# jinkyu032/TPDM

Hardware: NVIDIA B200
Metric: images/sec/box, SD3-M 1024^2 TPDM sampling (higher is better)
Workload: dtype bf16

## Files before the change

### include/tpdm_b200.h

```cpp
#ifndef TPDM_B200_H_
#define TPDM_B200_H_

#include <stddef.h>
#include <stdint.h>

#ifdef __cplusplus
extern "C" {
#endif

#define TPDM_ABI_VERSION 3

typedef enum tpdm_status {
  TPDM_OK = 0,
  TPDM_ERR_ARG = -1,
  TPDM_ERR_SHAPE = -2,
  TPDM_ERR_CUDA = -3,
  TPDM_ERR_STATE = -4,
  TPDM_ERR_NOMEM = -5
} tpdm_status;

typedef struct tpdm_config {
  int32_t num_layers;
  int32_t num_heads;
  int32_t head_dim;
// ... 198 lines not shown
int tpdm_vae_set_weights(tpdm_vae* vae, const tpdm_vae_weights* w);
size_t tpdm_vae_workspace_bytes(const tpdm_vae* vae, int latent_h, int latent_w);
int tpdm_vae_decode(tpdm_vae* vae, const float* latents, int apply_scaling, int batch, int latent_h, int latent_w,
                    void* workspace, size_t workspace_bytes, float* image, unsigned char* rgb, void* stream);

long long tpdm_launch_count(int reset);
int tpdm_profile_start(int max_records);
int tpdm_profile_stop(double* ms, double* flops, long long* count, int n_classes);
long long tpdm_profile_dropped(void);

int tpdm_gemm_bf16(const void* A, const void* W, const float* bias, const float* gate, void* out, int batch, int rows,
                   int N, int K, int epi, void* stream);
int tpdm_joint_attention(const void* qkv, void* out, int Bt, int S, int H, int dp, int head_dim, int q_rows, void* stream);
int tpdm_attention_redo_count(void);
long long tpdm_attention_redo_total(void);
int tpdm_conv3x3_nhwc(const void* x, const void* w, const float* bias, float* out, int batch, int g, int C, int N,
                      void* stream);
int tpdm_conv3x3_wgrad(const void* dyt, const void* x_shifted_nchw, float* dw, int samples, int g, int C, int M, void* stream);
int tpdm_ln_modulate(const float* x, const float* shift, const float* scale, int mod_stride, void* out_bf16, int batch,
                     int rows, int D, void* stream);

#ifdef __cplusplus
}
#endif
#endif
```

### tpdm_b200/_lib.py

```python
from __future__ import annotations

import ctypes as C
import os

HERE = os.path.dirname(os.path.abspath(__file__))
LIB_PATH = os.environ.get("TPDM_B200_LIB", os.path.join(HERE, "libtpdm_b200.so"))

c_float_p = C.POINTER(C.c_float)
vp = C.c_void_p

TPDM_OK, TPDM_ERR_ARG, TPDM_ERR_SHAPE, TPDM_ERR_CUDA, TPDM_ERR_STATE, TPDM_ERR_NOMEM = 0, -1, -2, -3, -4, -5


class TpdmConfig(C.Structure):
    _fields_ = [(n, C.c_int32) for n in (
        "num_layers", "num_heads", "head_dim", "joint_attention_dim", "pooled_projection_dim", "in_channels",
        "out_channels", "patch_size", "pos_embed_max_size", "qk_norm", "tpm_channels", "prediction_type", "relative")
    ] + [("min_sigma", C.c_float), ("epsilon", C.c_float), ("tpm_epsilon", C.c_float), ("dual_attention_mask", C.c_uint64)]


BLOCK_FIELDS = ("qkv_w", "qkv_b", "cqkv_w", "cqkv_b", "out_w", "out_b", "cout_w", "cout_b", "ff1_w", "ff1_b", "ff2_w",
                "ff2_b", "cff1_w", "cff1_b", "cff2_w", "cff2_b", "norm_q", "norm_k", "norm_added_q", "norm_added_k",
                "qkv2_w", "qkv2_b", "out2_w", "out2_b", "norm_q2", "norm_k2")

# ... 75 lines not shown
    "tpdm_rollout_shaping": (C.c_int, [vp, vp, vp, vp, vp, C.c_int, C.c_int, C.c_int, C.c_int, C.c_float, C.c_float, C.c_int, C.c_int,
                                       vp, vp, vp, vp, vp]),
    "tpdm_ppo_clip_loss": (C.c_int, [vp, vp, vp, vp, C.c_int, C.c_int, C.c_float, C.c_float, C.c_int, C.c_int, C.c_float, C.c_float, vp, vp, vp,
                                     vp, vp]),
    "tpdm_beta_logprob": (C.c_int, [vp, vp, C.c_int, C.c_int, C.c_float, C.c_float, C.c_int, C.c_int, C.c_float, vp, vp, vp]),
    "tpdm_adamw_step": (C.c_int, [vp, vp, vp, vp, C.c_longlong, C.c_float, C.c_float, C.c_float, C.c_float, C.c_float, C.c_float, C.c_int,
                                  C.c_float, vp, vp, C.c_longlong, vp, vp]),
    "tpdm_launch_count": (C.c_longlong, [C.c_int]),
    "tpdm_profile_start": (C.c_int, [C.c_int]),
    "tpdm_profile_dropped": (C.c_longlong, []),
    "tpdm_profile_stop": (C.c_int, [C.POINTER(C.c_double), C.POINTER(C.c_double), C.POINTER(C.c_longlong), C.c_int]),
    "tpdm_gemm_bf16": (C.c_int, [vp, vp, vp, vp, vp, C.c_int, C.c_int, C.c_int, C.c_int, C.c_int, vp]),
    "tpdm_joint_attention": (C.c_int, [vp, vp, C.c_int, C.c_int, C.c_int, C.c_int, C.c_int, C.c_int, vp]),
    "tpdm_attention_redo_count": (C.c_int, []),
    "tpdm_attention_redo_total": (C.c_longlong, []),
    "tpdm_conv3x3_nhwc": (C.c_int, [vp, vp, vp, vp, C.c_int, C.c_int, C.c_int, C.c_int, vp]),
    "tpdm_conv3x3_wgrad": (C.c_int, [vp, vp, vp, C.c_int, C.c_int, C.c_int, C.c_int, vp]),
    "tpdm_ln_modulate": (C.c_int, [vp, vp, vp, C.c_int, vp, C.c_int, C.c_int, C.c_int, vp]),
}

_lib = None


def load() -> C.CDLL:
    global _lib
    if _lib is None:
        if not os.path.exists(LIB_PATH):
            raise RuntimeError(f"{LIB_PATH} is missing: build it with `python -m tpdm_b200.build` "
                               "(tpdm_b200 has no CPU / PyTorch fallback)")
        lib = C.CDLL(LIB_PATH)
# ... 34 lines not shown
```

### tpdm_b200/csrc/api.cu

```cuda
#include <string.h>

#include <new>
#include <cstdlib>
#include <vector>

#include "host.h"
#include "kernels.h"

using namespace tpdm;

struct tpdm_ctx {
  tpdm_config cfg;
  tpdm_weights w;
  std::vector<tpdm_block_weights> blocks;
  bool has_weights = false, has_mmdit = false, has_tpm = false;
  int D = 0, dp = 0, Dp = 0, R = 0, device = 0;
  std::vector<int> mod_off;
  bool any_dual = false;
  bool dual(int i) const { return i < 64 && ((cfg.dual_attention_mask >> i) & 1ull) != 0; }
  int norm1_rows(int i) const { return (dual(i) ? 9 : 6) * D; }
};

namespace {

// ... 748 lines not shown
  TPDM_TRY(gemm_op_init(&op, A, K, static_cast<long long>(rows) * K, rows, batch, K, W, N, epi, out, static_cast<long long>(rows) * N, N, bias,
                        gate, N));
  return gemm_launch(&op, 1, static_cast<cudaStream_t>(stream));
}

int tpdm_joint_attention(const void* qkv, void* out, int Bt, int S, int H, int dp, int head_dim, int q_rows, void* stream) {
  TPDM_CHECK(qkv && out, TPDM_ERR_ARG, "tpdm_joint_attention: null argument");
  AttnOp op;
  TPDM_TRY(attn_op_init(&op, qkv, Bt, S, H, dp, head_dim, out));
  if (q_rows > 0 && q_rows < S) op.q_tiles = (q_rows + 127) / 128;
  return attn_launch(&op, static_cast<cudaStream_t>(stream));
}

int tpdm_attention_redo_count(void) { return attn_redo_count(); }
long long tpdm_attention_redo_total(void) { return attn_redo_total(); }

int tpdm_conv3x3_nhwc(const void* x, const void* w, const float* bias, float* out, int batch, int g, int C, int N, void* stream) {
  TPDM_CHECK(x && w && out, TPDM_ERR_ARG, "tpdm_conv3x3_nhwc: null argument");
  GemmOp op;
  TPDM_TRY(gemm_op_init_conv3x3(&op, x, batch, g, C, w, N, EPI_BIAS_F32, out, N, bias));
  return gemm_launch(&op, 1, static_cast<cudaStream_t>(stream));
}

int tpdm_conv3x3_wgrad(const void* dyt, const void* x_shifted_nchw, float* dw, int samples, int g, int C, int M, void* stream) {
  TPDM_CHECK(dyt && x_shifted_nchw && dw, TPDM_ERR_ARG, "tpdm_conv3x3_wgrad: null argument");
  GemmOp op;
  TPDM_TRY(gemm_op_init_conv3x3_wgrad(&op, dyt, x_shifted_nchw, samples, g, C, M, dw));
  return gemm_launch(&op, 1, static_cast<cudaStream_t>(stream));
}

// ... 9 lines not shown
```

### tpdm_b200/csrc/attention_tcgen05.cu

```cuda
#include <cuda_bf16.h>

#include <stdlib.h>

#include <type_traits>

#include "common.cuh"
#include "host.h"

namespace tpdm {

namespace {

constexpr int kFastThreads = 384;
constexpr int kQT = 128;
constexpr int kKT = 128;
constexpr int kChunk = 32;
constexpr int kKVStages = 2;
constexpr float kRescaleThreshold = 32.0f;
constexpr int kPolyEvery = 4;
#ifdef TPDM_ATTN_TRACE
__device__ long long g_attn_trace[3][2048];
#define ATRACE(role, idx)                                                                       \
  do {                                                                                          \
    if (trace_on && lane == 0 && (idx) < 2048) g_attn_trace[role][idx] = clock64();             \
  } while (0)
#define STRACE(e)                                                                               \
  do {                                                                                          \
    if (warp == 4) ATRACE(0, 8 * j + (e));                                                      \
  } while (0)
__device__ long long g_cta_trace[2][16];
#define CTRACE(idx)                                                                             \
  do {                                                                                          \
    if (ctr >= 0 && threadIdx.x == 128) g_cta_trace[ctr][idx] = clock64();                      \
  } while (0)
#else
#define ATRACE(role, idx)
#define STRACE(e)
#define CTRACE(idx)
#endif

__device__ unsigned long long g_redo_total;

template <int DP>
struct AttnSmem {
  static constexpr int kTile = kQT * DP * 2;
  static constexpr int kQOff = 0;
  static constexpr int kKOff = kTile;
  static constexpr int kVOff = kKOff + kKVStages * kTile;
  static constexpr int kBarOff = kVOff + kKVStages * kTile;
  static constexpr int kTotal = kBarOff + 256 + 1024;
  static constexpr uint32_t kTmemCols = DP == 64 ? 256 : 512;
  static constexpr uint32_t kSCol = 0;
  static constexpr uint32_t kPCol = 128;
  static constexpr uint32_t kOCol = 192;
};

template <int DP>
struct AttnBars {
  uint64_t *q_full, *k_full, *v_full, *k_empty, *v_empty, *s_full, *s_free, *p_full, *pv_done;
  uint32_t* tmem_slot;
  __device__ explicit AttnBars(uint8_t* smem) {
    uint64_t* bars = reinterpret_cast<uint64_t*>(smem + AttnSmem<DP>::kBarOff);
    q_full = bars + 0;
    k_full = bars + 1;
    v_full = k_full + kKVStages;
    k_empty = v_full + kKVStages;
    v_empty = k_empty + kKVStages;
    s_full = v_empty + kKVStages;
    s_free = s_full + 1;
    p_full = s_free + 1;
    pv_done = p_full + 2;
    tmem_slot = reinterpret_cast<uint32_t*>(pv_done + 1);
  }
  static constexpr int kCount = 1 + 4 * kKVStages + 5;
  __device__ void init(bool again, uint32_t s_free_count) const {
    if (again) {
      for (int i = 0; i < kCount; ++i) mbar_inval(q_full + i);
    }
    mbar_init(q_full, 1);
    for (int i = 0; i < kKVStages; ++i) {
      mbar_init(&k_full[i], 1);
      mbar_init(&v_full[i], 1);
      mbar_init(&k_empty[i], 1);
      mbar_init(&v_empty[i], 1);
    }
    mbar_init(s_full, 1);
    mbar_init(s_free, s_free_count);
    mbar_init(&p_full[0], 4);
    mbar_init(&p_full[1], 4);
    mbar_init(pv_done, 1);
    fence_barrier_init();
  }
};

// ... 35 lines not shown
    if (row_valid) {
      uint4* dst = reinterpret_cast<uint4*>(out + c * 32);
#pragma unroll
      for (int e = 0; e < 4; ++e) {
        uint4 w;
        w.x = pack_bf16x2(__uint_as_float(o[8 * e + 0]) * inv_l, __uint_as_float(o[8 * e + 1]) * inv_l);
        w.y = pack_bf16x2(__uint_as_float(o[8 * e + 2]) * inv_l, __uint_as_float(o[8 * e + 3]) * inv_l);
        w.z = pack_bf16x2(__uint_as_float(o[8 * e + 4]) * inv_l, __uint_as_float(o[8 * e + 5]) * inv_l);
        w.w = pack_bf16x2(__uint_as_float(o[8 * e + 6]) * inv_l, __uint_as_float(o[8 * e + 7]) * inv_l);
        dst[e] = w;
      }
    }
  }
}

template <int DP, bool kFast>
__device__ __forceinline__ void attn_cta(const AttnOp& A, uint8_t* smem, const int qt, const int h, const int b, int* redo_smem) {
  using L = AttnSmem<DP>;
  const AttnBars<DP> B(smem);
  uint64_t *const q_full = B.q_full, *const k_full = B.k_full, *const v_full = B.v_full, *const k_empty = B.k_empty,
                 *const v_empty = B.v_empty, *const s_full = B.s_full, *const s_free = B.s_free, *const p_full = B.p_full,
                 *const pv_done = B.pv_done;
  const int warp = threadIdx.x >> 5;
  const int lane = threadIdx.x & 31;
  const int q0 = qt * kQT;
  const int n_kv = (A.S + kKT - 1) / kKT;
#ifdef TPDM_ATTN_TRACE
  const int ctr = !kFast ? -1 : (qt == 5 && h == 3 && b == 0) ? 0 : (qt == 7 && h == 20 && b == 1) ? 1 : -1;
  const bool trace_on = ctr == 0;
#endif
  const uint32_t tmem_base = *B.tmem_slot;

  if (warp < 4) {
  if (warp == 0) {
    if (lane == 0) {
      mbar_arrive_expect_tx(q_full, L::kTile);
#pragma unroll
      for (int hh = 0; hh < DP / 64; ++hh) tma_load_4d(smem + L::kQOff + hh * (kQT * 128), &A.tmQ, q_full, hh * 64, h, q0, b);
      int stage = 0;
      uint32_t phase = 0;
      for (int j = 0; j < n_kv; ++j) {
        mbar_wait_backoff(&k_empty[stage], phase ^ 1);
        mbar_arrive_expect_tx(&k_full[stage], L::kTile);
#pragma unroll
        for (int hh = 0; hh < DP / 64; ++hh)
          tma_load_4d(smem + L::kKOff + stage * L::kTile + hh * (kKT * 128), &A.tmK, &k_full[stage], hh * 64, h, j * kKT, b);
        mbar_wait_backoff(&v_empty[stage], phase ^ 1);
        mbar_arrive_expect_tx(&v_full[stage], L::kTile);
#pragma unroll
        for (int hh = 0; hh < DP / 64; ++hh)
          tma_load_4d(smem + L::kVOff + stage * L::kTile + hh * (kKT * 128), &A.tmV, &v_full[stage], hh * 64, h, j * kKT, b);
        if (++stage == kKVStages) {
          stage = 0;
          phase ^= 1;
        }
      }
    }
  } else if (warp == 1) {
    constexpr uint32_t idesc_qk = make_idesc_bf16(kQT, kKT, false);
    const uint32_t q_base = smem_u32(smem + L::kQOff);
    mbar_wait(q_full, 0);
    for (int j = 0; j < n_kv; ++j) {
      const int stage = j % kKVStages;
      ATRACE(1, 4 * j);
      mbar_wait(&k_full[stage], (j / kKVStages) & 1);
      if (j >= 1) mbar_wait_backoff(s_free, (j - 1) & 1);
      tc_fence_after();
      ATRACE(1, 4 * j + 1);
      {
        const uint32_t k_base = smem_u32(smem + L::kKOff + stage * L::kTile);
        const uint64_t qdesc0 = make_smem_desc_sw128(q_base, 16, 1024), kdesc0 = make_smem_desc_sw128(k_base, 16, 1024);
#pragma unroll
        for (int ks = 0; ks < DP / 16; ++ks) {
          const uint32_t off = ((ks / 4) * (kQT * 128) + (ks % 4) * 32) >> 4;
          umma_ss_elect(tmem_base + L::kSCol, qdesc0 + off, kdesc0 + off, idesc_qk, ks != 0 ? 1u : 0u);
        }
        umma_commit_elect(s_full);
      }
      ATRACE(1, 4 * j + 2);
      __syncwarp();
    }
  } else if (warp == 3) {
    constexpr uint32_t idesc_pv = make_idesc_bf16(kQT, DP, true);
    for (int j = 0; j < n_kv; ++j) {
      const int stage = j % kKVStages;
      ATRACE(2, 4 * j);
#pragma unroll
      for (int half = 0; half < 2; ++half) {
        mbar_wait_backoff(&p_full[half], j & 1);
        if (half == 0) mbar_wait(&v_full[stage], (j / kKVStages) & 1);
        tc_fence_after();
        if (half == 0) ATRACE(2, 4 * j + 1);
        {
          const uint32_t v_base = smem_u32(smem + L::kVOff + stage * L::kTile);
          const uint64_t vdesc0 = make_smem_desc_sw128(v_base, kKT * 128, 1024);
#pragma unroll
          for (int k4 = 0; k4 < kKT / 32; ++k4) {
            const int ks = half * (kKT / 32) + k4;
            umma_ts_elect(tmem_base + L::kOCol, tmem_base + L::kPCol + ks * 8, vdesc0 + ks * (2048 >> 4), idesc_pv, (j | ks) != 0 ? 1u : 0u);
          }
          if (half == 1) umma_commit_elect(pv_done);
        }
        __syncwarp();
      }
      ATRACE(2, 4 * j + 2);
      __syncwarp();
    }
  }
  } else if (kFast) {
    __shared__ float xch[2][kQT];
    __shared__ int bump[2][kQT];
    const int q = warp & 3, half = (warp - 4) >> 2;
    const uint32_t lane_off = static_cast<uint32_t>(q * 32) << 16;
    const uint32_t s_tmem = tmem_base + lane_off + L::kSCol + half * 64;
    const uint32_t p_tmem = tmem_base + lane_off + L::kPCol + half * 32;
    const uint32_t o_tmem = tmem_base + lane_off + L::kOCol + half * (DP / 2);
    const int rowi = q * 32 + lane;
    const float scale = A.scale_log2;
    const uint64_t scale2 = pack_f32x2(scale, scale);
    constexpr float kHard = 1.8446744073709552e19f, kPolyMax = 127.f;
    uint64_t la = pack_f32x2(0.f, 0.f), lb = pack_f32x2(0.f, 0.f);
    float pmax = -INFINITY;
    bool hard = false;
    float applied = 0.f;
    if (half == 0) {
      bump[0][q * 32 + lane] = 0;
      bump[1][q * 32 + lane] = 0;
    }
    auto mask16 = [&](const int c, uint32_t (&v)[16], const int valid) {
      if (valid < kKT) {
#pragma unroll
        for (int e = 0; e < 16; ++e)
          if (half * 64 + c * 16 + e >= valid) v[e] = 0xff800000u;
      }
    };
    mbar_wait(s_full, 0);
    tc_fence_after();
    float m_ref;
    {
      const int valid0 = A.S < kKT ? A.S : kKT;
      float mx = -INFINITY;
#pragma unroll 1
      for (int c = 0; c < 4; ++c) {
        uint32_t v[16];
        tmem_ld_32x16(s_tmem + c * 16, v);
        tmem_wait_ld();
        mask16(c, v, valid0);
#pragma unroll
        for (int e = 0; e < 16; e += 2) mx = fmax3(mx, __uint_as_float(v[e]), __uint_as_float(v[e + 1]));
      }
      xch[half][rowi] = mx * scale;
      asm volatile("bar.sync 1, 256;" ::: "memory");
      m_ref = fmaxf(xch[0][rowi], xch[1][rowi]);
      asm volatile("bar.sync 1, 256;" ::: "memory");
    }
    CTRACE(3);
    uint64_t negm2 = pack_f32x2(-m_ref, -m_ref);
    auto exp16 = [&](const uint32_t (&v)[16], uint32_t (&pk)[8]) {
#pragma unroll
      for (int i = 0; i < 8; ++i) {
        float x0, x1, p0, p1;
        unpack_f32x2(ffma2(pack_f32x2(__uint_as_float(v[2 * i]), __uint_as_float(v[2 * i + 1])), scale2, negm2), x0, x1);
        const bool poly = i % kPolyEvery == kPolyEvery - 1;
        if (poly) pmax = fmax3(pmax, x0, x1);
        exp2_pair(x0, x1, poly, p0, p1);
        if (i & 1) lb = fadd2(lb, pack_f32x2(p0, p1));
        else la = fadd2(la, pack_f32x2(p0, p1));
        pk[i] = pack_bf16x2(p0, p1);
      }
    };
    auto row_sum = [&]() {
      float a0, a1, b0, b1;
      unpack_f32x2(la, a0, a1);
      unpack_f32x2(lb, b0, b1);
      return (a0 + a1) + (b0 + b1);
    };
    auto tile = [&](const int j, auto masked_tag) {
      constexpr bool kMasked = decltype(masked_tag)::value;
      const int valid = A.S - j * kKT;
      STRACE(0);
      hard = hard || pmax > kPolyMax;
      mbar_wait(s_full, j & 1);
      tc_fence_after();
      if (warp == 4 && lane == 0) mbar_arrive(&k_empty[j % kKVStages]);
      STRACE(1);
      uint32_t va[16], vb[16], pk[8];
      tmem_ld_32x16(s_tmem, va);
      tmem_ld_32x16(s_tmem + 16, vb);
      if ((j & 3) == 3) {
        const int c = j >> 2;
        const float lsum = row_sum();
        const float total = __int_as_float(bump[c & 1][rowi]);
        const bool over = !(lsum <= 16777216.f);
        hard = hard || !(lsum <= kHard);
        if (__any_sync(0xffffffffu, over || total > applied)) {
          const float e = total > applied ? total - applied : 0.f;
          if (over && lsum <= kHard)
            atomicMax(&bump[(c + 1) & 1][rowi],
                      __float_as_int(fmaxf(total, applied) + fmaxf(static_cast<float>((__float_as_int(lsum) >> 23) - 127) - e, 0.f)));
          const float m_new = m_ref + e;
          const float alpha = exp2_approx(m_ref - m_new);
          m_ref = m_new;
          applied = fmaxf(total, applied);
          negm2 = pack_f32x2(-m_ref, -m_ref);
          mbar_wait(pv_done, (j - 1) & 1);
          tc_fence_after();
#pragma unroll 1
          for (int cc = 0; cc < DP / 32; ++cc) {
            uint32_t o[16];
            tmem_ld_32x16(o_tmem + cc * 16, o);
            tmem_wait_ld();
#pragma unroll
            for (int i = 0; i < 16; ++i) o[i] = __float_as_uint(__uint_as_float(o[i]) * alpha);
            tmem_st_32x16(o_tmem + cc * 16, o);
          }
          const uint64_t alpha2 = pack_f32x2(alpha, alpha);
          la = fmul2(la, alpha2);
          lb = fmul2(lb, alpha2);
        }
      }
      tmem_wait_ld();
      STRACE(2);
      if (kMasked) {
        mask16(0, va, valid);
        mask16(1, vb, valid);
      }
      exp16(va, pk);
      if (j > 0) {
        mbar_wait(pv_done, (j - 1) & 1);
        tc_fence_after();
        if (warp == 4 && lane == 0) mbar_arrive(&v_empty[(j - 1) % kKVStages]);
      }
      tmem_st_32x8(p_tmem, pk);
      tmem_ld_32x16(s_tmem + 32, va);
      STRACE(3);
      exp16(vb, pk);
      tmem_st_32x8(p_tmem + 8, pk);
      tmem_ld_32x16(s_tmem + 48, vb);
      tmem_wait_ld();
      tc_fence_before();
      __syncwarp();
      if (lane == 0) mbar_arrive(s_free);
      STRACE(4);
      if (kMasked) {
        mask16(2, va, valid);
        mask16(3, vb, valid);
      }
      exp16(va, pk);
      tmem_st_32x8(p_tmem + 16, pk);
      exp16(vb, pk);
      tmem_st_32x8(p_tmem + 24, pk);
      tmem_wait_st();
      tc_fence_before();
      __syncwarp();
      if (lane == 0) mbar_arrive(&p_full[half]);
      STRACE(5);
    };
    for (int j = 0; j < n_kv - 1; ++j) tile(j, std::false_type{});
    tile(n_kv - 1, std::true_type{});
    CTRACE(4);
    const float lh = row_sum();
    if (!(lh <= kHard) || pmax > kPolyMax) hard = true;
    if (hard) *redo_smem = 1;
    xch[half][rowi] = lh;
    asm volatile("bar.sync 1, 256;" ::: "memory");
    const float inv_l = 1.0f / (xch[0][rowi] + xch[1][rowi]);
    mbar_wait(pv_done, (n_kv - 1) & 1);
    tc_fence_after();
    const int row = q0 + rowi;
    store_o<DP / 2>(o_tmem, inv_l,
                    A.out + (static_cast<long long>(b) * A.S + row) * (static_cast<long long>(A.H) * DP) + h * DP + half * (DP / 2), row < A.S);
  } else if (warp < 8) {
    const int q = warp & 3;
    const uint32_t lane_off = static_cast<uint32_t>(q * 32) << 16;
    const uint32_t s_tmem = tmem_base + lane_off + L::kSCol;
    const uint32_t p_tmem = tmem_base + lane_off + L::kPCol;
    const uint32_t o_tmem = tmem_base + lane_off + L::kOCol;
    const float scale = A.scale_log2;
    const uint64_t scale2 = pack_f32x2(scale, scale);
    float m_used = -INFINITY;
    uint64_t l2 = pack_f32x2(0.f, 0.f);

    auto exp_half = [&](const uint32_t (&v)[32], uint32_t (&pk)[16], uint64_t negm2, const int half) {
#pragma unroll
      for (int ii = 0; ii < 8; ++ii) {
        const int i = half * 8 + ii;
// ... 106 lines not shown
          tmem_wait_st();
          tc_fence_before();
          __syncwarp();
          if (lane == 0) mbar_arrive(&p_full[c == kLast ? 1 : 0]);
        }
      };
      do_chunk(0, va, vb);
      do_chunk(1, vb, va);
      do_chunk(2, va, vb);
      do_chunk(3, vb, va);
    }
    float l_lo, l_hi;
    unpack_f32x2(l2, l_lo, l_hi);
    mbar_wait(pv_done, (n_kv - 1) & 1);
    tc_fence_after();
    const int row = q0 + q * 32 + lane;
    store_o<DP>(o_tmem, 1.0f / (l_lo + l_hi), A.out + (static_cast<long long>(b) * A.S + row) * (static_cast<long long>(A.H) * DP) + h * DP,
                row < A.S);
  }

  __syncwarp();
  tc_fence_before();
  __syncthreads();
}

template <int DP>
__global__ void __launch_bounds__(kFastThreads, DP == 64 ? 2 : 1) joint_attention_fast_kernel(const __grid_constant__ AttnOp A) {
  using L = AttnSmem<DP>;
  pdl_launch_dependents();
  uint8_t* smem = attn_smem_base();
  const AttnBars<DP> B(smem);
  __shared__ int redo_smem;
  const int warp = threadIdx.x >> 5, lane = threadIdx.x & 31;
#ifdef TPDM_ATTN_TRACE
  const int ctr = (blockIdx.x == 5 && blockIdx.y == 3 && blockIdx.z == 0) ? 0 : (blockIdx.x == 7 && blockIdx.y == 20 && blockIdx.z == 1) ? 1 : -1;
  if (ctr >= 0 && threadIdx.x == 128) {
    long long t;
    asm volatile("mov.u64 %0, %%globaltimer;" : "=l"(t));
    g_cta_trace[ctr][7] = t;
  }
#endif
  CTRACE(0);
  if (warp == 0 && lane == 0) {
    tma_prefetch_desc(&A.tmQ);
    tma_prefetch_desc(&A.tmK);
    tma_prefetch_desc(&A.tmV);
  }
  if (warp == 1 && lane == 0) B.init(false, 8);
  if (threadIdx.x == 0) redo_smem = 0;
  pdl_wait();
  CTRACE(1);
  const int cta_id = (blockIdx.z * gridDim.y + blockIdx.y) * gridDim.x + blockIdx.x;
  const bool idle = (A.skip != nullptr && *A.skip != 0) || (A.bmask != nullptr && A.bmask[blockIdx.z % A.bslots] == 0);
  if (idle) {
    if (A.redo != nullptr && threadIdx.x == 0) A.redo[cta_id] = 0;
    return;
  }
  if (warp == 2) {
    tmem_alloc<L::kTmemCols>(B.tmem_slot);
    tmem_relinquish();
  }
  tc_fence_before();
  __syncthreads();
  tc_fence_after();
  CTRACE(2);
  attn_cta<DP, true>(A, smem, blockIdx.x, blockIdx.y, blockIdx.z, &redo_smem);
  CTRACE(5);
  const int redo = redo_smem;
  if (redo != 0) {
    if (threadIdx.x == 0) atomicAdd(&g_redo_total, 1ull);
    if (warp == 1 && lane == 0) B.init(true, 4);
    tc_fence_before();
    __syncthreads();
    tc_fence_after();
    attn_cta<DP, false>(A, smem, blockIdx.x, blockIdx.y, blockIdx.z, nullptr);
  }
  if (A.redo != nullptr && threadIdx.x == 0) A.redo[cta_id] = redo;
  if (warp == 2) tmem_dealloc<L::kTmemCols>(*B.tmem_slot);
#ifdef TPDM_ATTN_TRACE
  CTRACE(6);
  if (ctr >= 0 && threadIdx.x == 128) {
    long long t;
    asm volatile("mov.u64 %0, %%globaltimer;" : "=l"(t));
    g_cta_trace[ctr][8] = t;
  }
#endif
}

constexpr size_t kRedoCapacity = size_t(1) << 20;
int* redo_slice(size_t n) {
  static int* buf = nullptr;
  static size_t cursor = 0;
  if (n > kRedoCapacity) return nullptr;
  if (buf == nullptr && cudaMalloc(&buf, kRedoCapacity * sizeof(int)) != cudaSuccess) {
    buf = nullptr;
    (void)cudaGetLastError();
    return nullptr;
  }
  if (cursor + n > kRedoCapacity) cursor = 0;
  int* p = buf + cursor;
  cursor += n;
  return p;
}

const int* g_last_redo = nullptr;
int g_last_redo_n = 0;

template <int DP>
int attn_launch_impl(const AttnOp& op, cudaStream_t stream) {
  static bool attr_set = false;
  if (!attr_set) {
    TPDM_CUDA_OK(cudaFuncSetAttribute(joint_attention_fast_kernel<DP>, cudaFuncAttributeMaxDynamicSharedMemorySize, AttnSmem<DP>::kTotal));
    attr_set = true;
  }
  dim3 grid(op.q_tiles, op.H, op.Bt);
  g_last_redo = op.redo;
  g_last_redo_n = op.q_tiles * op.H * op.Bt;
  const double q_rows = op.q_tiles * kQT < op.S ? op.q_tiles * kQT : op.S;
  prof_begin(1, 4.0 * op.Bt * op.H * q_rows * op.S * op.head_dim, stream);
  TPDM_CUDA_OK(launch_pdl(joint_attention_fast_kernel<DP>, grid, dim3(kFastThreads), AttnSmem<DP>::kTotal, stream, op));
  prof_end(stream);
  count_launch();
  TPDM_CUDA_OK(cudaGetLastError());
  return 0;
}

}

int attn_op_init(AttnOp* op, const void* qkv, int Bt, int S, int H, int dp, int head_dim, void* out) {
  *op = AttnOp{};
  TPDM_CHECK(dp == 64 || dp == 128, TPDM_ERR_SHAPE, "attention: padded head dim %d must be 64 or 128", dp);
  TPDM_CHECK(head_dim > 0 && head_dim <= dp, TPDM_ERR_SHAPE, "attention: head_dim %d exceeds padded %d", head_dim, dp);
// ... 6 lines not shown
  op->q_tiles = (S + kQT - 1) / kQT;
  op->scale_log2 = 1.4426950408889634f / sqrtf(static_cast<float>(head_dim));
  op->out = reinterpret_cast<__nv_bfloat16*>(out);
  op->redo = redo_slice(static_cast<size_t>(op->q_tiles) * H * Bt);
  const uint64_t row = static_cast<uint64_t>(3) * H * dp;
  uint64_t dims[4] = {static_cast<uint64_t>(dp), static_cast<uint64_t>(H), static_cast<uint64_t>(S), static_cast<uint64_t>(Bt)};
  uint64_t strides[3] = {static_cast<uint64_t>(dp) * 2, row * 2, row * S * 2};
  uint32_t box[4] = {64, 1, kQT, 1};
  const __nv_bfloat16* base = reinterpret_cast<const __nv_bfloat16*>(qkv);
  TPDM_TRY(encode_tmap_bf16(&op->tmQ, base, 4, dims, strides, box));
  TPDM_TRY(encode_tmap_bf16(&op->tmK, base + static_cast<size_t>(H) * dp, 4, dims, strides, box));
  TPDM_TRY(encode_tmap_bf16(&op->tmV, base + static_cast<size_t>(2) * H * dp, 4, dims, strides, box));
  return 0;
}

long long attn_redo_total() {
  unsigned long long v = 0;
  if (cudaDeviceSynchronize() != cudaSuccess) return -2;
  if (cudaMemcpyFromSymbol(&v, g_redo_total, sizeof(v)) != cudaSuccess) return -2;
  return static_cast<long long>(v);
}

int attn_redo_count() {
  if (g_last_redo == nullptr) return -1;
  static int* host = nullptr;
  static int host_n = 0;
  if (host_n < g_last_redo_n) {
    free(host);
    host = static_cast<int*>(malloc(sizeof(int) * g_last_redo_n));
    host_n = g_last_redo_n;
  }
  if (cudaDeviceSynchronize() != cudaSuccess) return -2;
  if (cudaMemcpy(host, g_last_redo, sizeof(int) * g_last_redo_n, cudaMemcpyDeviceToHost) != cudaSuccess) return -2;
  int n = 0;
  for (int i = 0; i < g_last_redo_n; ++i) n += host[i] != 0;
  return n;
}

#ifdef TPDM_ATTN_TRACE
extern "C" int tpdm_attn_cta_trace_read(long long* host) {
  return cudaMemcpyFromSymbol(host, g_cta_trace, sizeof(long long) * 32) == cudaSuccess ? 0 : -1;
}
extern "C" int tpdm_attn_trace_read(long long* host, int n) {
  return cudaMemcpyFromSymbol(host, g_attn_trace, sizeof(long long) * (n < 3 * 2048 ? n : 3 * 2048)) == cudaSuccess ? 0 : -1;
}
#endif

int attn_launch(const AttnOp* op_in, cudaStream_t stream) {
  AttnOp op_copy = *op_in;
  op_copy.skip = skip_flag();
  op_copy.bmask = batch_mask();
  op_copy.bslots = batch_mask_slots();
  const AttnOp* op = &op_copy;
  return op->dp == 64 ? attn_launch_impl<64>(*op, stream) : attn_launch_impl<128>(*op, stream);
}

// ... 2 lines not shown
```

### tpdm_b200/csrc/host.h

```cpp
#pragma once
#include <cuda.h>
#include <cuda_bf16.h>
#include <utility>
#include <cuda_runtime.h>
#include <stdint.h>
#include <stdio.h>

#include <string>

#include "../../include/tpdm_b200.h"

namespace tpdm {

void set_last_error(const std::string& msg);
int fail(int code, const char* fmt, ...);

#define TPDM_CUDA_OK(expr)                                                                           \
  do {                                                                                               \
    cudaError_t _e = (expr);                                                                         \
    if (_e != cudaSuccess)                                                                           \
      return ::tpdm::fail(TPDM_ERR_CUDA, "%s failed: %s (%s:%d)", #expr, cudaGetErrorString(_e), __FILE__, __LINE__); \
  } while (0)

#define TPDM_CHECK(cond, code, ...)                     \
// ... 83 lines not shown
struct alignas(64) AttnOp {
  CUtensorMap tmQ, tmK, tmV;
  int S, H, Bt, dp;
  int q_tiles, head_dim;
  float scale_log2;
  const int* skip;
  const int* bmask = nullptr;
  int bslots = 1;
  __nv_bfloat16* out;
  int* redo = nullptr;
};
int attn_op_init(AttnOp* op, const void* qkv, int Bt, int S, int H, int dp, int head_dim, void* out);
int attn_launch(const AttnOp* op, cudaStream_t stream);
long long attn_redo_total();
int attn_redo_count();

}
```

Baseline: 2.254.

## Make joint attention kernel persistent with double-buffered Q across work items

The attention kernel now launches a persistent grid sized to resident CTAs. Each CTA loops over strided (q-tile, head, batch) items and double-buffers the Q tile, so the next item's Q and K/V loads overlap the current item's softmax and epilogue. Barrier phases are carried across items, masked batches are skipped per item, and redo flags become a per-CTA bitmask that is replayed after the fast pass. This removes per-CTA launch, TMEM allocation and pipeline fill costs. In exchange it doubles Q shared memory, adds cross-item phase bookkeeping, and can unbalance work when items do not divide evenly across CTAs.

```diff
diff --git a/include/tpdm_b200.h b/include/tpdm_b200.h
--- a/include/tpdm_b200.h
+++ b/include/tpdm_b200.h
@@ -236,6 +236,7 @@
 int tpdm_joint_attention(const void* qkv, void* out, int Bt, int S, int H, int dp, int head_dim, int q_rows, void* stream);
 int tpdm_attention_redo_count(void);
 long long tpdm_attention_redo_total(void);
+int tpdm_attention_set_max_ctas(int n);
 int tpdm_conv3x3_nhwc(const void* x, const void* w, const float* bias, float* out, int batch, int g, int C, int N,
                       void* stream);
 int tpdm_conv3x3_wgrad(const void* dyt, const void* x_shifted_nchw, float* dw, int samples, int g, int C, int M, void* stream);
diff --git a/tpdm_b200/_lib.py b/tpdm_b200/_lib.py
--- a/tpdm_b200/_lib.py
+++ b/tpdm_b200/_lib.py
@@ -113,6 +113,7 @@
     "tpdm_joint_attention": (C.c_int, [vp, vp, C.c_int, C.c_int, C.c_int, C.c_int, C.c_int, C.c_int, vp]),
     "tpdm_attention_redo_count": (C.c_int, []),
     "tpdm_attention_redo_total": (C.c_longlong, []),
+    "tpdm_attention_set_max_ctas": (C.c_int, [C.c_int]),
     "tpdm_conv3x3_nhwc": (C.c_int, [vp, vp, vp, vp, C.c_int, C.c_int, C.c_int, C.c_int, vp]),
     "tpdm_conv3x3_wgrad": (C.c_int, [vp, vp, vp, C.c_int, C.c_int, C.c_int, C.c_int, vp]),
     "tpdm_ln_modulate": (C.c_int, [vp, vp, vp, C.c_int, vp, C.c_int, C.c_int, C.c_int, vp]),
diff --git a/tpdm_b200/csrc/api.cu b/tpdm_b200/csrc/api.cu
--- a/tpdm_b200/csrc/api.cu
+++ b/tpdm_b200/csrc/api.cu
@@ -786,6 +786,7 @@
 
 int tpdm_attention_redo_count(void) { return attn_redo_count(); }
 long long tpdm_attention_redo_total(void) { return attn_redo_total(); }
+int tpdm_attention_set_max_ctas(int n) { return attn_set_max_ctas(n); }
 
 int tpdm_conv3x3_nhwc(const void* x, const void* w, const float* bias, float* out, int batch, int g, int C, int N, void* stream) {
   TPDM_CHECK(x && w && out, TPDM_ERR_ARG, "tpdm_conv3x3_nhwc: null argument");
diff --git a/tpdm_b200/csrc/attention_tcgen05.cu b/tpdm_b200/csrc/attention_tcgen05.cu
--- a/tpdm_b200/csrc/attention_tcgen05.cu
+++ b/tpdm_b200/csrc/attention_tcgen05.cu
@@ -16,27 +16,34 @@
 constexpr int kKT = 128;
 constexpr int kChunk = 32;
 constexpr int kKVStages = 2;
+constexpr int kMaxItemsPerCta = 4096;
 constexpr float kRescaleThreshold = 32.0f;
 constexpr int kPolyEvery = 4;
 #ifdef TPDM_ATTN_TRACE
+constexpr int kTraceItem = 1;
 __device__ long long g_attn_trace[3][2048];
 #define ATRACE(role, idx)                                                                       \
   do {                                                                                          \
-    if (trace_on && lane == 0 && (idx) < 2048) g_attn_trace[role][idx] = clock64();             \
+    if (ctr == 0 && n == kTraceItem && lane == 0 && (idx) < 2048) g_attn_trace[role][idx] = clock64(); \
   } while (0)
 #define STRACE(e)                                                                               \
   do {                                                                                          \
     if (warp == 4) ATRACE(0, 8 * j + (e));                                                      \
   } while (0)
-__device__ long long g_cta_trace[2][16];
+__device__ long long g_cta_trace[2][32];
 #define CTRACE(idx)                                                                             \
   do {                                                                                          \
     if (ctr >= 0 && threadIdx.x == 128) g_cta_trace[ctr][idx] = clock64();                      \
+  } while (0)
+#define CTRACE_ITEM(e)                                                                          \
+  do {                                                                                          \
+    if (n < 8) CTRACE(8 + 3 * n + (e));                                                         \
   } while (0)
 #else
 #define ATRACE(role, idx)
 #define STRACE(e)
 #define CTRACE(idx)
+#define CTRACE_ITEM(e)
 #endif
 
 __device__ unsigned long long g_redo_total;
@@ -45,7 +52,7 @@
 struct AttnSmem {
   static constexpr int kTile = kQT * DP * 2;
   static constexpr int kQOff = 0;
-  static constexpr int kKOff = kTile;
+  static constexpr int kKOff = 2 * kTile;
   static constexpr int kVOff = kKOff + kKVStages * kTile;
   static constexpr int kBarOff = kVOff + kKVStages * kTile;
   static constexpr int kTotal = kBarOff + 256 + 1024;
@@ -57,12 +64,13 @@
 
 template <int DP>
 struct AttnBars {
-  uint64_t *q_full, *k_full, *v_full, *k_empty, *v_empty, *s_full, *s_free, *p_full, *pv_done;
+  uint64_t *q_full, *q_empty, *k_full, *v_full, *k_empty, *v_empty, *s_full, *s_free, *p_full, *pv_done;
   uint32_t* tmem_slot;
   __device__ explicit AttnBars(uint8_t* smem) {
     uint64_t* bars = reinterpret_cast<uint64_t*>(smem + AttnSmem<DP>::kBarOff);
     q_full = bars + 0;
-    k_full = bars + 1;
+    q_empty = q_full + 2;
+    k_full = q_empty + 2;
     v_full = k_full + kKVStages;
     k_empty = v_full + kKVStages;
     v_empty = k_empty + kKVStages;
@@ -72,12 +80,15 @@
     pv_done = p_full + 2;
     tmem_slot = reinterpret_cast<uint32_t*>(pv_done + 1);
   }
-  static constexpr int kCount = 1 + 4 * kKVStages + 5;
+  static constexpr int kCount = 4 + 4 * kKVStages + 5;
   __device__ void init(bool again, uint32_t s_free_count) const {
     if (again) {
       for (int i = 0; i < kCount; ++i) mbar_inval(q_full + i);
     }
-    mbar_init(q_full, 1);
+    for (int i = 0; i < 2; ++i) {
+      mbar_init(&q_full[i], 1);
+      mbar_init(&q_empty[i], 1);
+    }
     for (int i = 0; i < kKVStages; ++i) {
       mbar_init(&k_full[i], 1);
       mbar_init(&v_full[i], 1);
@@ -143,97 +154,134 @@
   }
 }
 
+struct AttnItem {
+  int qt, h, b;
+  bool active;
+};
+__device__ __forceinline__ AttnItem attn_item(const AttnOp& A, const int item) {
+  AttnItem it;
+  it.qt = item % A.q_tiles;
+  const int bh = item / A.q_tiles;
+  it.h = bh % A.H;
+  it.b = bh / A.H;
+  it.active = A.bmask == nullptr || A.bmask[it.b % A.bslots] != 0;
+  return it;
+}
+
 template <int DP, bool kFast>
-__device__ __forceinline__ void attn_cta(const AttnOp& A, uint8_t* smem, const int qt, const int h, const int b, int* redo_smem) {
+__device__ __forceinline__ void attn_cta(const AttnOp& A, uint8_t* smem, const int item0, const int stride, const int n_items,
+                                         uint32_t* redo_bits) {
   using L = AttnSmem<DP>;
   const AttnBars<DP> B(smem);
-  uint64_t *const q_full = B.q_full, *const k_full = B.k_full, *const v_full = B.v_full, *const k_empty = B.k_empty,
-                 *const v_empty = B.v_empty, *const s_full = B.s_full, *const s_free = B.s_free, *const p_full = B.p_full,
-                 *const pv_done = B.pv_done;
+  uint64_t *const q_full = B.q_full, *const q_empty = B.q_empty, *const k_full = B.k_full, *const v_full = B.v_full,
+                 *const k_empty = B.k_empty, *const v_empty = B.v_empty, *const s_full = B.s_full, *const s_free = B.s_free,
+                 *const p_full = B.p_full, *const pv_done = B.pv_done;
   const int warp = threadIdx.x >> 5;
   const int lane = threadIdx.x & 31;
-  const int q0 = qt * kQT;
   const int n_kv = (A.S + kKT - 1) / kKT;
 #ifdef TPDM_ATTN_TRACE
-  const int ctr = !kFast ? -1 : (qt == 5 && h == 3 && b == 0) ? 0 : (qt == 7 && h == 20 && b == 1) ? 1 : -1;
-  const bool trace_on = ctr == 0;
+  const int ctr = !kFast ? -1 : blockIdx.x == 0 ? 0 : blockIdx.x == gridDim.x - 1 ? 1 : -1;
 #endif
   const uint32_t tmem_base = *B.tmem_slot;
 
   if (warp < 4) {
   if (warp == 0) {
     if (lane == 0) {
-      mbar_arrive_expect_tx(q_full, L::kTile);
-#pragma unroll
-      for (int hh = 0; hh < DP / 64; ++hh) tma_load_4d(smem + L::kQOff + hh * (kQT * 128), &A.tmQ, q_full, hh * 64, h, q0, b);
       int stage = 0;
       uint32_t phase = 0;
-      for (int j = 0; j < n_kv; ++j) {
-        mbar_wait_backoff(&k_empty[stage], phase ^ 1);
-        mbar_arrive_expect_tx(&k_full[stage], L::kTile);
+      int n = 0;
+      for (int i = 0; i < n_items; ++i) {
+        const AttnItem it = attn_item(A, item0 + i * stride);
+        if (!it.active) continue;
+        const int qb = n & 1;
+        mbar_wait_backoff(&q_empty[qb], ((n >> 1) & 1) ^ 1);
+        mbar_arrive_expect_tx(&q_full[qb], L::kTile);
 #pragma unroll
         for (int hh = 0; hh < DP / 64; ++hh)
-          tma_load_4d(smem + L::kKOff + stage * L::kTile + hh * (kKT * 128), &A.tmK, &k_full[stage], hh * 64, h, j * kKT, b);
-        mbar_wait_backoff(&v_empty[stage], phase ^ 1);
-        mbar_arrive_expect_tx(&v_full[stage], L::kTile);
-#pragma unroll
-        for (int hh = 0; hh < DP / 64; ++hh)
-          tma_load_4d(smem + L::kVOff + stage * L::kTile + hh * (kKT * 128), &A.tmV, &v_full[stage], hh * 64, h, j * kKT, b);
-        if (++stage == kKVStages) {
-          stage = 0;
-          phase ^= 1;
-        }
-      }
+          tma_load_4d(smem + L::kQOff + qb * L::kTile + hh * (kQT * 128), &A.tmQ, &q_full[qb], hh * 64, it.h, it.qt * kQT, it.b);
+        for (int j = 0; j < n_kv; ++j) {
+          mbar_wait_backoff(&k_empty[stage], phase ^ 1);
+          mbar_arrive_expect_tx(&k_full[stage], L::kTile);
+#pragma unroll
+          for (int hh = 0; hh < DP / 64; ++hh)
+            tma_load_4d(smem + L::kKOff + stage * L::kTile + hh * (kKT * 128), &A.tmK, &k_full[stage], hh * 64, it.h, j * kKT, it.b);
+          mbar_wait_backoff(&v_empty[stage], phase ^ 1);
+          mbar_arrive_expect_tx(&v_full[stage], L::kTile);
+#pragma unroll
+          for (int hh = 0; hh < DP / 64; ++hh)
+            tma_load_4d(smem + L::kVOff + stage * L::kTile + hh * (kKT * 128), &A.tmV, &v_full[stage], hh * 64, it.h, j * kKT, it.b);
+          if (++stage == kKVStages) {
+            stage = 0;
+            phase ^= 1;
+          }
+        }
+        ++n;
+      }
+      for (int m = n > 2 ? n - 2 : 0; m < n; ++m) mbar_wait_backoff(&q_empty[m & 1], (m >> 1) & 1);
     }
   } else if (warp == 1) {
     constexpr uint32_t idesc_qk = make_idesc_bf16(kQT, kKT, false);
-    const uint32_t q_base = smem_u32(smem + L::kQOff);
-    mbar_wait(q_full, 0);
-    for (int j = 0; j < n_kv; ++j) {
-      const int stage = j % kKVStages;
-      ATRACE(1, 4 * j);
-      mbar_wait(&k_full[stage], (j / kKVStages) & 1);
-      if (j >= 1) mbar_wait_backoff(s_free, (j - 1) & 1);
-      tc_fence_after();
-      ATRACE(1, 4 * j + 1);
-      {
-        const uint32_t k_base = smem_u32(smem + L::kKOff + stage * L::kTile);
-        const uint64_t qdesc0 = make_smem_desc_sw128(q_base, 16, 1024), kdesc0 = make_smem_desc_sw128(k_base, 16, 1024);
-#pragma unroll
-        for (int ks = 0; ks < DP / 16; ++ks) {
-          const uint32_t off = ((ks / 4) * (kQT * 128) + (ks % 4) * 32) >> 4;
-          umma_ss_elect(tmem_base + L::kSCol, qdesc0 + off, kdesc0 + off, idesc_qk, ks != 0 ? 1u : 0u);
-        }
-        umma_commit_elect(s_full);
-      }
-      ATRACE(1, 4 * j + 2);
-      __syncwarp();
+    int n = 0;
+    for (int i = 0; i < n_items; ++i) {
+      if (!__all_sync(0xffffffffu, attn_item(A, item0 + i * stride).active)) continue;
+      const int qb = n & 1;
+      const uint32_t q_base = smem_u32(smem + L::kQOff + qb * L::kTile);
+      mbar_wait(&q_full[qb], (n >> 1) & 1);
+      for (int j = 0; j < n_kv; ++j) {
+        const int g = n * n_kv + j;
+        const int stage = g % kKVStages;
+        ATRACE(1, 4 * j);
+        mbar_wait(&k_full[stage], (g / kKVStages) & 1);
+        if (g >= 1) mbar_wait_backoff(s_free, (g - 1) & 1);
+        tc_fence_after();
+        ATRACE(1, 4 * j + 1);
+        {
+          const uint32_t k_base = smem_u32(smem + L::kKOff + stage * L::kTile);
+          const uint64_t qdesc0 = make_smem_desc_sw128(q_base, 16, 1024), kdesc0 = make_smem_desc_sw128(k_base, 16, 1024);
+#pragma unroll
+          for (int ks = 0; ks < DP / 16; ++ks) {
+            const uint32_t off = ((ks / 4) * (kQT * 128) + (ks % 4) * 32) >> 4;
+            umma_ss_elect(tmem_base + L::kSCol, qdesc0 + off, kdesc0 + off, idesc_qk, ks != 0 ? 1u : 0u);
+          }
+          umma_commit_elect(s_full);
+          if (j == n_kv - 1) umma_commit_elect(&q_empty[qb]);
+        }
+        ATRACE(1, 4 * j + 2);
+        __syncwarp();
+      }
+      ++n;
     }
   } else if (warp == 3) {
     constexpr uint32_t idesc_pv = make_idesc_bf16(kQT, DP, true);
-    for (int j = 0; j < n_kv; ++j) {
-      const int stage = j % kKVStages;
-      ATRACE(2, 4 * j);
-#pragma unroll
-      for (int half = 0; half < 2; ++half) {
-        mbar_wait_backoff(&p_full[half], j & 1);
-        if (half == 0) mbar_wait(&v_full[stage], (j / kKVStages) & 1);
-        tc_fence_after();
-        if (half == 0) ATRACE(2, 4 * j + 1);
-        {
-          const uint32_t v_base = smem_u32(smem + L::kVOff + stage * L::kTile);
-          const uint64_t vdesc0 = make_smem_desc_sw128(v_base, kKT * 128, 1024);
-#pragma unroll
-          for (int k4 = 0; k4 < kKT / 32; ++k4) {
-            const int ks = half * (kKT / 32) + k4;
-            umma_ts_elect(tmem_base + L::kOCol, tmem_base + L::kPCol + ks * 8, vdesc0 + ks * (2048 >> 4), idesc_pv, (j | ks) != 0 ? 1u : 0u);
+    int n = 0;
+    for (int i = 0; i < n_items; ++i) {
+      if (!__all_sync(0xffffffffu, attn_item(A, item0 + i * stride).active)) continue;
+      for (int j = 0; j < n_kv; ++j) {
+        const int g = n * n_kv + j;
+        const int stage = g % kKVStages;
+        ATRACE(2, 4 * j);
+#pragma unroll
+        for (int half = 0; half < 2; ++half) {
+          mbar_wait_backoff(&p_full[half], g & 1);
+          if (half == 0) mbar_wait(&v_full[stage], (g / kKVStages) & 1);
+          tc_fence_after();
+          if (half == 0) ATRACE(2, 4 * j + 1);
+          {
+            const uint32_t v_base = smem_u32(smem + L::kVOff + stage * L::kTile);
+            const uint64_t vdesc0 = make_smem_desc_sw128(v_base, kKT * 128, 1024);
+#pragma unroll
+            for (int k4 = 0; k4 < kKT / 32; ++k4) {
+              const int ks = half * (kKT / 32) + k4;
+              umma_ts_elect(tmem_base + L::kOCol, tmem_base + L::kPCol + ks * 8, vdesc0 + ks * (2048 >> 4), idesc_pv, (j | ks) != 0 ? 1u : 0u);
+            }
+            if (half == 1) umma_commit_elect(pv_done);
           }
-          if (half == 1) umma_commit_elect(pv_done);
-        }
+          __syncwarp();
+        }
+        ATRACE(2, 4 * j + 2);
         __syncwarp();
       }
-      ATRACE(2, 4 * j + 2);
-      __syncwarp();
+      ++n;
     }
   }
   } else if (kFast) {
@@ -248,14 +296,14 @@
     const float scale = A.scale_log2;
     const uint64_t scale2 = pack_f32x2(scale, scale);
     constexpr float kHard = 1.8446744073709552e19f, kPolyMax = 127.f;
-    uint64_t la = pack_f32x2(0.f, 0.f), lb = pack_f32x2(0.f, 0.f);
-    float pmax = -INFINITY;
-    bool hard = false;
-    float applied = 0.f;
-    if (half == 0) {
-      bump[0][q * 32 + lane] = 0;
-      bump[1][q * 32 + lane] = 0;
-    }
+    uint64_t la, lb;
+    float pmax;
+    bool hard;
+    float applied;
+    float m_ref;
+    uint64_t negm2;
+    int n = 0;
+    int g0 = 0;
     auto mask16 = [&](const int c, uint32_t (&v)[16], const int valid) {
       if (valid < kKT) {
 #pragma unroll
@@ -263,28 +311,6 @@
           if (half * 64 + c * 16 + e >= valid) v[e] = 0xff800000u;
       }
     };
-    mbar_wait(s_full, 0);
-    tc_fence_after();
-    float m_ref;
-    {
-      const int valid0 = A.S < kKT ? A.S : kKT;
-      float mx = -INFINITY;
-#pragma unroll 1
-      for (int c = 0; c < 4; ++c) {
-        uint32_t v[16];
-        tmem_ld_32x16(s_tmem + c * 16, v);
-        tmem_wait_ld();
-        mask16(c, v, valid0);
-#pragma unroll
-        for (int e = 0; e < 16; e += 2) mx = fmax3(mx, __uint_as_float(v[e]), __uint_as_float(v[e + 1]));
-      }
-      xch[half][rowi] = mx * scale;
-      asm volatile("bar.sync 1, 256;" ::: "memory");
-      m_ref = fmaxf(xch[0][rowi], xch[1][rowi]);
-      asm volatile("bar.sync 1, 256;" ::: "memory");
-    }
-    CTRACE(3);
-    uint64_t negm2 = pack_f32x2(-m_ref, -m_ref);
     auto exp16 = [&](const uint32_t (&v)[16], uint32_t (&pk)[8]) {
 #pragma unroll
       for (int i = 0; i < 8; ++i) {
@@ -308,10 +334,11 @@
       constexpr bool kMasked = decltype(masked_tag)::value;
       const int valid = A.S - j * kKT;
       STRACE(0);
+      const int g = g0 + j;
       hard = hard || pmax > kPolyMax;
-      mbar_wait(s_full, j & 1);
+      mbar_wait(s_full, g & 1);
       tc_fence_after();
-      if (warp == 4 && lane == 0) mbar_arrive(&k_empty[j % kKVStages]);
+      if (warp == 4 && lane == 0) mbar_arrive(&k_empty[g % kKVStages]);
       STRACE(1);
       uint32_t va[16], vb[16], pk[8];
       tmem_ld_32x16(s_tmem, va);
@@ -332,7 +359,7 @@
           m_ref = m_new;
           applied = fmaxf(total, applied);
           negm2 = pack_f32x2(-m_ref, -m_ref);
-          mbar_wait(pv_done, (j - 1) & 1);
+          mbar_wait(pv_done, (g - 1) & 1);
           tc_fence_after();
 #pragma unroll 1
           for (int cc = 0; cc < DP / 32; ++cc) {
@@ -355,10 +382,10 @@
         mask16(1, vb, valid);
       }
       exp16(va, pk);
-      if (j > 0) {
-        mbar_wait(pv_done, (j - 1) & 1);
+      if (g > 0) {
+        mbar_wait(pv_done, (g - 1) & 1);
         tc_fence_after();
-        if (warp == 4 && lane == 0) mbar_arrive(&v_empty[(j - 1) % kKVStages]);
+        if (warp == 4 && lane == 0) mbar_arrive(&v_empty[(g - 1) % kKVStages]);
       }
       tmem_st_32x8(p_tmem, pk);
       tmem_ld_32x16(s_tmem + 32, va);
@@ -385,20 +412,57 @@
       if (lane == 0) mbar_arrive(&p_full[half]);
       STRACE(5);
     };
-    for (int j = 0; j < n_kv - 1; ++j) tile(j, std::false_type{});
-    tile(n_kv - 1, std::true_type{});
-    CTRACE(4);
-    const float lh = row_sum();
-    if (!(lh <= kHard) || pmax > kPolyMax) hard = true;
-    if (hard) *redo_smem = 1;
-    xch[half][rowi] = lh;
-    asm volatile("bar.sync 1, 256;" ::: "memory");
-    const float inv_l = 1.0f / (xch[0][rowi] + xch[1][rowi]);
-    mbar_wait(pv_done, (n_kv - 1) & 1);
-    tc_fence_after();
-    const int row = q0 + rowi;
-    store_o<DP / 2>(o_tmem, inv_l,
-                    A.out + (static_cast<long long>(b) * A.S + row) * (static_cast<long long>(A.H) * DP) + h * DP + half * (DP / 2), row < A.S);
+    for (int i = 0; i < n_items; ++i) {
+      const AttnItem it = attn_item(A, item0 + i * stride);
+      if (!__all_sync(0xffffffffu, it.active)) continue;
+      g0 = __shfl_sync(0xffffffffu, n * n_kv, 0);
+      la = pack_f32x2(0.f, 0.f);
+      lb = pack_f32x2(0.f, 0.f);
+      pmax = -INFINITY;
+      hard = false;
+      applied = 0.f;
+      bump[half][rowi] = 0;
+      mbar_wait(s_full, g0 & 1);
+      tc_fence_after();
+      {
+        const int valid0 = A.S < kKT ? A.S : kKT;
+        float mx = -INFINITY;
+#pragma unroll 1
+        for (int c = 0; c < 4; ++c) {
+          uint32_t v[16];
+          tmem_ld_32x16(s_tmem + c * 16, v);
+          tmem_wait_ld();
+          mask16(c, v, valid0);
+#pragma unroll
+          for (int e = 0; e < 16; e += 2) mx = fmax3(mx, __uint_as_float(v[e]), __uint_as_float(v[e + 1]));
+        }
+        xch[half][rowi] = mx * scale;
+        asm volatile("bar.sync 1, 256;" ::: "memory");
+        m_ref = fmaxf(xch[0][rowi], xch[1][rowi]);
+        asm volatile("bar.sync 1, 256;" ::: "memory");
+      }
+      CTRACE_ITEM(0);
+      negm2 = pack_f32x2(-m_ref, -m_ref);
+      for (int j = 0; j < n_kv - 1; ++j) tile(j, std::false_type{});
+      tile(n_kv - 1, std::true_type{});
+      CTRACE_ITEM(1);
+      const float lh = row_sum();
+      if (!(lh <= kHard) || pmax > kPolyMax) hard = true;
+      if (hard) atomicOr(&redo_bits[i >> 5], 1u << (i & 31));
+      xch[half][rowi] = lh;
+      asm volatile("bar.sync 1, 256;" ::: "memory");
+      const float inv_l = 1.0f / (xch[0][rowi] + xch[1][rowi]);
+      mbar_wait(pv_done, (g0 + n_kv - 1) & 1);
+      tc_fence_after();
+      const int row = it.qt * kQT + rowi;
+      store_o<DP / 2>(o_tmem, inv_l,
+                      A.out + (static_cast<long long>(it.b) * A.S + row) * (static_cast<long long>(A.H) * DP) + it.h * DP + half * (DP / 2),
+                      row < A.S);
+      tc_fence_before();
+      asm volatile("bar.sync 1, 256;" ::: "memory");
+      CTRACE_ITEM(2);
+      ++n;
+    }
   } else if (warp < 8) {
     const int q = warp & 3;
     const uint32_t lane_off = static_cast<uint32_t>(q * 32) << 16;
@@ -535,8 +599,9 @@
     unpack_f32x2(l2, l_lo, l_hi);
     mbar_wait(pv_done, (n_kv - 1) & 1);
     tc_fence_after();
-    const int row = q0 + q * 32 + lane;
-    store_o<DP>(o_tmem, 1.0f / (l_lo + l_hi), A.out + (static_cast<long long>(b) * A.S + row) * (static_cast<long long>(A.H) * DP) + h * DP,
+    const AttnItem it = attn_item(A, item0);
+    const int row = it.qt * kQT + q * 32 + lane;
+    store_o<DP>(o_tmem, 1.0f / (l_lo + l_hi), A.out + (static_cast<long long>(it.b) * A.S + row) * (static_cast<long long>(A.H) * DP) + it.h * DP,
                 row < A.S);
   }
 
@@ -551,14 +616,17 @@
   pdl_launch_dependents();
   uint8_t* smem = attn_smem_base();
   const AttnBars<DP> B(smem);
-  __shared__ int redo_smem;
+  __shared__ uint32_t redo_bits[kMaxItemsPerCta / 32];
   const int warp = threadIdx.x >> 5, lane = threadIdx.x & 31;
+  const int items = A.q_tiles * A.H * A.Bt;
+  const int n_items = (items - 1 - static_cast<int>(blockIdx.x)) / static_cast<int>(gridDim.x) + 1;
 #ifdef TPDM_ATTN_TRACE
-  const int ctr = (blockIdx.x == 5 && blockIdx.y == 3 && blockIdx.z == 0) ? 0 : (blockIdx.x == 7 && blockIdx.y == 20 && blockIdx.z == 1) ? 1 : -1;
+  const int ctr = blockIdx.x == 0 ? 0 : blockIdx.x == gridDim.x - 1 ? 1 : -1;
   if (ctr >= 0 && threadIdx.x == 128) {
     long long t;
     asm volatile("mov.u64 %0, %%globaltimer;" : "=l"(t));
-    g_cta_trace[ctr][7] = t;
+    g_cta_trace[ctr][5] = t;
+    g_cta_trace[ctr][7] = n_items;
   }
 #endif
   CTRACE(0);
@@ -568,13 +636,12 @@
     tma_prefetch_desc(&A.tmV);
   }
   if (warp == 1 && lane == 0) B.init(false, 8);
-  if (threadIdx.x == 0) redo_smem = 0;
+  for (int w = threadIdx.x; w < (n_items + 31) / 32; w += kFastThreads) redo_bits[w] = 0;
   pdl_wait();
   CTRACE(1);
-  const int cta_id = (blockIdx.z * gridDim.y + blockIdx.y) * gridDim.x + blockIdx.x;
-  const bool idle = (A.skip != nullptr && *A.skip != 0) || (A.bmask != nullptr && A.bmask[blockIdx.z % A.bslots] == 0);
-  if (idle) {
-    if (A.redo != nullptr && threadIdx.x == 0) A.redo[cta_id] = 0;
+  if (A.skip != nullptr && *A.skip != 0) {
+    if (A.redo != nullptr)
+      for (int i = threadIdx.x; i < n_items; i += kFastThreads) A.redo[blockIdx.x + i * gridDim.x] = 0;
     return;
   }
   if (warp == 2) {
@@ -585,25 +652,28 @@
   __syncthreads();
   tc_fence_after();
   CTRACE(2);
-  attn_cta<DP, true>(A, smem, blockIdx.x, blockIdx.y, blockIdx.z, &redo_smem);
-  CTRACE(5);
-  const int redo = redo_smem;
-  if (redo != 0) {
-    if (threadIdx.x == 0) atomicAdd(&g_redo_total, 1ull);
+  attn_cta<DP, true>(A, smem, blockIdx.x, gridDim.x, n_items, redo_bits);
+  CTRACE(3);
+  int redone = 0;
+  for (int i = 0; i < n_items; ++i) {
+    if (((redo_bits[i >> 5] >> (i & 31)) & 1u) == 0) continue;
+    ++redone;
     if (warp == 1 && lane == 0) B.init(true, 4);
     tc_fence_before();
     __syncthreads();
     tc_fence_after();
-    attn_cta<DP, false>(A, smem, blockIdx.x, blockIdx.y, blockIdx.z, nullptr);
-  }
-  if (A.redo != nullptr && threadIdx.x == 0) A.redo[cta_id] = redo;
+    attn_cta<DP, false>(A, smem, blockIdx.x + i * gridDim.x, 0, 1, nullptr);
+  }
+  if (redone != 0 && threadIdx.x == 0) atomicAdd(&g_redo_total, static_cast<unsigned long long>(redone));
+  if (A.redo != nullptr)
+    for (int i = threadIdx.x; i < n_items; i += kFastThreads) A.redo[blockIdx.x + i * gridDim.x] = (redo_bits[i >> 5] >> (i & 31)) & 1u;
   if (warp == 2) tmem_dealloc<L::kTmemCols>(*B.tmem_slot);
 #ifdef TPDM_ATTN_TRACE
-  CTRACE(6);
+  CTRACE(4);
   if (ctr >= 0 && threadIdx.x == 128) {
     long long t;
     asm volatile("mov.u64 %0, %%globaltimer;" : "=l"(t));
-    g_cta_trace[ctr][8] = t;
+    g_cta_trace[ctr][6] = t;
   }
 #endif
 }
@@ -627,16 +697,27 @@
 const int* g_last_redo = nullptr;
 int g_last_redo_n = 0;
 
+int g_max_ctas = 0;
+
 template <int DP>
 int attn_launch_impl(const AttnOp& op, cudaStream_t stream) {
-  static bool attr_set = false;
-  if (!attr_set) {
+  static int resident = 0;
+  if (resident == 0) {
     TPDM_CUDA_OK(cudaFuncSetAttribute(joint_attention_fast_kernel<DP>, cudaFuncAttributeMaxDynamicSharedMemorySize, AttnSmem<DP>::kTotal));
-    attr_set = true;
-  }
-  dim3 grid(op.q_tiles, op.H, op.Bt);
+    TPDM_CUDA_OK(cudaFuncSetAttribute(joint_attention_fast_kernel<DP>, cudaFuncAttributePreferredSharedMemoryCarveout, cudaSharedmemCarveoutMaxShared));
+    int per_sm = 0;
+    TPDM_CUDA_OK(cudaOccupancyMaxActiveBlocksPerMultiprocessor(&per_sm, joint_attention_fast_kernel<DP>, kFastThreads, AttnSmem<DP>::kTotal));
+    TPDM_CHECK(per_sm > 0, TPDM_ERR_CUDA, "attention: the dp = %d kernel does not fit on an SM", DP);
+    resident = per_sm * num_sms();
+  }
+  const int items = op.q_tiles * op.H * op.Bt;
+  int ctas = g_max_ctas > 0 ? g_max_ctas : resident;
+  if (ctas > items) ctas = items;
+  const int min_ctas = (items + kMaxItemsPerCta - 1) / kMaxItemsPerCta;
+  if (ctas < min_ctas) ctas = min_ctas;
+  dim3 grid(ctas);
   g_last_redo = op.redo;
-  g_last_redo_n = op.q_tiles * op.H * op.Bt;
+  g_last_redo_n = items;
   const double q_rows = op.q_tiles * kQT < op.S ? op.q_tiles * kQT : op.S;
   prof_begin(1, 4.0 * op.Bt * op.H * q_rows * op.S * op.head_dim, stream);
   TPDM_CUDA_OK(launch_pdl(joint_attention_fast_kernel<DP>, grid, dim3(kFastThreads), AttnSmem<DP>::kTotal, stream, op));
@@ -673,6 +754,12 @@
   return 0;
 }
 
+int attn_set_max_ctas(int n) {
+  TPDM_CHECK(n >= 0, TPDM_ERR_ARG, "tpdm_attention_set_max_ctas: %d < 0", n);
+  g_max_ctas = n;
+  return 0;
+}
+
 long long attn_redo_total() {
   unsigned long long v = 0;
   if (cudaDeviceSynchronize() != cudaSuccess) return -2;
@@ -698,7 +785,7 @@
 
 #ifdef TPDM_ATTN_TRACE
 extern "C" int tpdm_attn_cta_trace_read(long long* host) {
-  return cudaMemcpyFromSymbol(host, g_cta_trace, sizeof(long long) * 32) == cudaSuccess ? 0 : -1;
+  return cudaMemcpyFromSymbol(host, g_cta_trace, sizeof(long long) * 64) == cudaSuccess ? 0 : -1;
 }
 extern "C" int tpdm_attn_trace_read(long long* host, int n) {
   return cudaMemcpyFromSymbol(host, g_attn_trace, sizeof(long long) * (n < 3 * 2048 ? n : 3 * 2048)) == cudaSuccess ? 0 : -1;
diff --git a/tpdm_b200/csrc/host.h b/tpdm_b200/csrc/host.h
--- a/tpdm_b200/csrc/host.h
+++ b/tpdm_b200/csrc/host.h
@@ -121,5 +121,6 @@
 int attn_launch(const AttnOp* op, cudaStream_t stream);
 long long attn_redo_total();
 int attn_redo_count();
+int attn_set_max_ctas(int n);
 
 }
```

After: 2.110, median of 6. -6.4%, worse.
